# guy3540/Acoustic_Locating_VQ-VAE

Hardware: AMD Instinct MI355X
Metric: spectrograms/sec (train step), speech VQ-VAE default config (higher is better)
Workload: dtype x3mx_hb

## Files before the change

acoustic_locating_vq-vae_amd/csrc/pack_weights.hip:

```cpp
#include "alvq_common.h"
#include "bf16_common.h"
#include "f16mx_common.h"
#include "nlc_host.h"

namespace alvq {

constexpr int PB_MAX = 32;
struct PackDesc {
  const float* w;
  u16* wp;
  int M, C, KW, layout, Mp, Cp, blk0, ctiles;
};
struct PackBatch {
  PackDesc d[PB_MAX];
  int n;
  long plane[PB_MAX];
};

template <int PLANES>
__device__ __forceinline__ void pack_store8(u16* wp, long plane, long row_off, int c, const float (&v)[8]) {
  const long o = row_off + c;
  if (PLANES == 3) {
    unsigned h[4], qh[2], ql[2];
    fx_split<8>(v, fx_pow2(FX_E_W), fx_pow2(FX_E_W - FX_LO_SHIFT), h, qh, ql);
    *(u32x4*)(wp + o) = u32x4{h[0], h[1], h[2], h[3]};
    unsigned char* q = (unsigned char*)(wp + plane) + row_off * 2 + fx_q_off(c);
    *(u32x2*)q = u32x2{qh[0], qh[1]};
    *(u32x2*)(q + 32) = u32x2{ql[0], ql[1]};
    return;
  }
  u32x4 hi;
#pragma unroll
  for (int e = 0; e < 4; ++e) hi[e] = f2bf_pk(v[2 * e], v[2 * e + 1]);
  *(u32x4*)(wp + o) = hi;
  if (PLANES == 2) {
    u32x4 lo;
#pragma unroll
    for (int e = 0; e < 4; ++e) {
      const float h0 = __uint_as_float(hi[e] << 16), h1 = __uint_as_float(hi[e] & 0xffff0000u);
      lo[e] = f2bf_pk(v[2 * e] - h0, v[2 * e + 1] - h1);
    }
    *(u32x4*)(wp + plane + o) = lo;
  }
}

template <int PLANES>
__global__ __launch_bounds__(256) void pack_weights_batch_kernel(PackBatch b) {
  __shared__ float tile[3][32][65];
  if (PLANES == 3) fx_saturating_conversions();
  int di = 0;
  for (int i = 1; i < b.n; ++i)
    if ((int)blockIdx.x >= b.d[i].blk0) di = i;
  const PackDesc& d = b.d[di];
  const int lb = blockIdx.x - d.blk0;
  const int m0 = (lb / d.ctiles) * 32, c0 = (lb % d.ctiles) * 64;
  const int KW = d.KW, tid = threadIdx.x;
  if (d.layout == ALVQ_W_OIK) {
    const int run = 64 * KW;
#pragma unroll 4
    for (int e = tid; e < 32 * run; e += 256) {
      const int mr = e / run, j = e - mr * run, c = j / KW, t = j - c * KW;
      const int m = m0 + mr;
      tile[t][mr][c] = (m < d.M && c0 + c < d.C) ? d.w[((long)m * d.C + c0) * KW + j] : 0.f;
    }
  } else {
    const int run = 32 * KW;
#pragma unroll 4
    for (int e = tid; e < 64 * run; e += 256) {
      const int cc = e / run, j = e - cc * run, mr = j / KW, k = j - mr * KW;
      const int c = c0 + cc;
      tile[KW - 1 - k][mr][cc] = (c < d.C && m0 + mr < d.M) ? d.w[((long)c * d.M + m0) * KW + j] : 0.f;
    }
  }
  __syncthreads();
  const int mr = tid >> 3, cg = (tid & 7) * 8;
  for (int t = 0; t < KW; ++t) {
    float v[8];
#pragma unroll
    for (int e = 0; e < 8; ++e) v[e] = tile[t][mr][cg + e];
    pack_store8<PLANES>(d.wp, b.plane[di], ((long)t * d.Mp + m0 + mr) * d.Cp, c0 + cg, v);
  }
}

constexpr int AP_MAX = 24;
struct AdamPackDesc {
  float* w; const float* g; float* m; float* v;
  u16* oik; u16* iok;
  int dim0, dim1, KW, blk0, tiles1;
  int oik_Mp, oik_Cp, iok_Mp, iok_Cp;
};
struct AdamPackBatch {
  AdamPackDesc d[AP_MAX];
  int n;
  const float* sc;
  const float* skip;
  float beta1, beta2, eps;
};

template <int PLANES>
__global__ __launch_bounds__(256) void adam_pack_batch_kernel(AdamPackBatch b) {
  __shared__ float tile[3][32][65];
  if (b.skip && *b.skip != 0.f) return;
  if (PLANES == 3) fx_saturating_conversions();
  int di = 0;
  for (int i = 1; i < b.n; ++i)
    if ((int)blockIdx.x >= b.d[i].blk0) di = i;
  const AdamPackDesc& d = b.d[di];
  const int lb = blockIdx.x - d.blk0;
  const int r0 = (lb / d.tiles1) * 32, q0 = (lb % d.tiles1) * 64;
  const int KW = d.KW, tid = threadIdx.x;
  const float lr_bc1 = b.sc[0], bc2_sqrt = b.sc[1], gscale = b.sc[2];
  const float beta1 = b.beta1, beta2 = b.beta2, eps = b.eps;
  const int run = 64 * KW;
  if (q0 + 64 <= d.dim1 && ((d.dim1 * KW) & 3) == 0) {
#pragma unroll 2
    for (int e4 = tid; e4 < 8 * run; e4 += 256) {
      const int e = 4 * e4, rr = e / run, j = e - rr * run;
      f32x4 wn = {0.f, 0.f, 0.f, 0.f};
      if (r0 + rr < d.dim0) {
        const long i = ((long)(r0 + rr) * d.dim1 + q0) * KW + j;
        const f32x4 g4 = *(const f32x4*)(d.g + i), m4 = *(const f32x4*)(d.m + i), v4 = *(const f32x4*)(d.v + i), w4 = *(const f32x4*)(d.w + i);
        f32x4 mo, vo;
#pragma unroll
        for (int q = 0; q < 4; ++q) {
          const float gr = g4[q] * gscale;
          const float mm = m4[q] + (gr - m4[q]) * (1.f - beta1);
          const float vv = v4[q] * beta2 + (1.f - beta2) * gr * gr;
          const float denom = sqrtf(vv) / bc2_sqrt + eps;
          mo[q] = mm;
          vo[q] = vv;
          wn[q] = w4[q] - lr_bc1 * (mm / denom);
        }
        *(f32x4*)(d.m + i) = mo;
        *(f32x4*)(d.v + i) = vo;
        *(f32x4*)(d.w + i) = wn;
      }
#pragma unroll
      for (int q = 0; q < 4; ++q) {
        const int jj = j + q, qq = jj / KW, t = jj - qq * KW;
        tile[t][rr][qq] = wn[q];
      }
    }
  } else {
#pragma unroll 2
    for (int e = tid; e < 32 * run; e += 256) {
      const int rr = e / run, j = e - rr * run, qq = j / KW, t = j - qq * KW;
      float wn = 0.f;
      if (r0 + rr < d.dim0 && q0 + qq < d.dim1) {
        const long i = ((long)(r0 + rr) * d.dim1 + q0) * KW + j;
        const float gr = d.g[i] * gscale;
        const float m0 = d.m[i], v0 = d.v[i];
        const float mm = m0 + (gr - m0) * (1.f - beta1);
        const float vv = v0 * beta2 + (1.f - beta2) * gr * gr;
        const float denom = sqrtf(vv) / bc2_sqrt + eps;
        d.m[i] = mm;
        d.v[i] = vv;
        wn = d.w[i] - lr_bc1 * (mm / denom);
        d.w[i] = wn;
      }
      tile[t][rr][qq] = wn;
    }
  }
  __syncthreads();
  if (d.oik) {
    const int mr = tid >> 3, cg = (tid & 7) * 8;
    const long plane = (long)KW * d.oik_Mp * d.oik_Cp;
    for (int t = 0; t < KW; ++t) {
      float v[8];
#pragma unroll
      for (int e = 0; e < 8; ++e) v[e] = tile[t][mr][cg + e];
      pack_store8<PLANES>(d.oik, plane, ((long)t * d.oik_Mp + r0 + mr) * d.oik_Cp, q0 + cg, v);
    }
  }
  if (d.iok) {
    const int mr = tid >> 2, cg = (tid & 3) * 8;
    const long plane = (long)KW * d.iok_Mp * d.iok_Cp;
    for (int t = 0; t < KW; ++t) {
      float v[8];
#pragma unroll
      for (int e = 0; e < 8; ++e) v[e] = tile[KW - 1 - t][cg + e][mr];
      pack_store8<PLANES>(d.iok, plane, ((long)t * d.iok_Mp + q0 + mr) * d.iok_Cp, r0 + cg, v);
    }
  }
}

constexpr int AS_MAX = 48;
struct AdamSegs {
  long lo[AS_MAX], hi[AS_MAX];
  int blk0[AS_MAX];
  int n;
};
__global__ __launch_bounds__(256) void adam_segments_kernel(float* p, const float* g, float* m, float* v, AdamSegs s, const float* sc,
                                                            float beta1, float beta2, float eps, const float* skip) {
  if (skip && *skip != 0.f) return;
  int si = 0;
  for (int i = 1; i < s.n; ++i)
    if ((int)blockIdx.x >= s.blk0[i]) si = i;
  const float lr_bc1 = sc[0], bc2_sqrt = sc[1], gscale = sc[2];
  const long base = s.lo[si] + (long)(blockIdx.x - s.blk0[si]) * 1024;
#pragma unroll
  for (int k = 0; k < 4; ++k) {
    const long e = base + k * 256 + threadIdx.x;
    if (e >= s.hi[si]) return;
    const float gr = g[e] * gscale;
    const float mm = m[e] + (gr - m[e]) * (1.f - beta1);
    const float vv = v[e] * beta2 + (1.f - beta2) * gr * gr;
    const float denom = sqrtf(vv) / bc2_sqrt + eps;
    m[e] = mm;
    v[e] = vv;
    p[e] = p[e] - lr_bc1 * (mm / denom);
  }
}

}

using namespace alvq;

extern "C" int alvq_pack_weights_bf16_batch(const alvq_pack_desc* descs, int n, int planes, void* stream) {
  ALVQ_REQUIRE(descs && n > 0, ALVQ_EINVAL, "alvq_pack_weights_bf16_batch: no descriptors");
  ALVQ_REQUIRE(planes >= 1 && planes <= 3, ALVQ_EINVAL, "alvq_pack_weights_bf16_batch: planes=%d (1, 2 or 3)", planes);
  for (int i = 0; i < n; ++i) {
    const alvq_pack_desc& s = descs[i];
    ALVQ_REQUIRE(s.w && s.wp, ALVQ_EINVAL, "alvq_pack_weights_bf16_batch: null pointer in descriptor %d", i);
    ALVQ_REQUIRE(s.M > 0 && s.C > 0 && (s.KW == 1 || s.KW == 3), ALVQ_EINVAL, "alvq_pack_weights_bf16_batch: bad dims in descriptor %d", i);
    ALVQ_REQUIRE(s.w_layout == ALVQ_W_OIK || s.w_layout == ALVQ_W_IOK, ALVQ_EINVAL, "alvq_pack_weights_bf16_batch: w_layout in descriptor %d", i);
  }
  for (int i0 = 0; i0 < n; i0 += PB_MAX) {
    PackBatch b{};
    b.n = n - i0 < PB_MAX ? n - i0 : PB_MAX;
    int blocks = 0;
    for (int i = 0; i < b.n; ++i) {
      const alvq_pack_desc& s = descs[i0 + i];
      PackDesc& d = b.d[i];
      d.w = s.w; d.wp = (u16*)s.wp; d.M = s.M; d.C = s.C; d.KW = s.KW; d.layout = s.w_layout;
      d.Mp = pad_to(s.M, WP_ROWS); d.Cp = pad_to(s.C, TB_K);
      d.blk0 = blocks; d.ctiles = d.Cp / 64;
      b.plane[i] = (long)s.KW * d.Mp * d.Cp;
      blocks += (d.Mp / 32) * d.ctiles;
    }
    if (planes == 1) hipLaunchKernelGGL(pack_weights_batch_kernel<1>, dim3(blocks), dim3(256), 0, (hipStream_t)stream, b);
    else if (planes == 2) hipLaunchKernelGGL(pack_weights_batch_kernel<2>, dim3(blocks), dim3(256), 0, (hipStream_t)stream, b);
    else hipLaunchKernelGGL(pack_weights_batch_kernel<3>, dim3(blocks), dim3(256), 0, (hipStream_t)stream, b);
    int rc = check_launch("alvq_pack_weights_bf16_batch");
    if (rc) return rc;
  }
  return ALVQ_OK;
}

extern "C" int alvq_adam_pack_batch(const alvq_adam_pack_desc* descs, int n, int planes, const float* scalars, float beta1,
                                    float beta2, float eps, const float* skip, void* stream) {
  ALVQ_REQUIRE(descs && n > 0 && scalars, ALVQ_EINVAL, "alvq_adam_pack_batch: no descriptors / scalars");
  ALVQ_REQUIRE(planes >= 1 && planes <= 3, ALVQ_EINVAL, "alvq_adam_pack_batch: planes=%d (1, 2 or 3)", planes);
  for (int i = 0; i < n; ++i) {
    const alvq_adam_pack_desc& s = descs[i];
    ALVQ_REQUIRE(s.w && s.g && s.m && s.v, ALVQ_EINVAL, "alvq_adam_pack_batch: null pointer in descriptor %d", i);
    ALVQ_REQUIRE(s.dim0 > 0 && s.dim1 > 0 && (s.KW == 1 || s.KW == 3), ALVQ_EINVAL, "alvq_adam_pack_batch: bad dims in descriptor %d", i);
  }
  for (int i0 = 0; i0 < n; i0 += AP_MAX) {
    AdamPackBatch b{};
    b.n = n - i0 < AP_MAX ? n - i0 : AP_MAX;
    b.sc = scalars; b.skip = skip; b.beta1 = beta1; b.beta2 = beta2; b.eps = eps;
    int blocks = 0;
    for (int i = 0; i < b.n; ++i) {
      const alvq_adam_pack_desc& s = descs[i0 + i];
      AdamPackDesc& d = b.d[i];
      d.w = s.w; d.g = s.g; d.m = s.m; d.v = s.v; d.oik = (u16*)s.wp_oik; d.iok = (u16*)s.wp_iok;
      d.dim0 = s.dim0; d.dim1 = s.dim1; d.KW = s.KW;
      d.oik_Mp = pad_to(s.dim0, WP_ROWS); d.oik_Cp = pad_to(s.dim1, TB_K);
      d.iok_Mp = pad_to(s.dim1, WP_ROWS); d.iok_Cp = pad_to(s.dim0, TB_K);
      d.blk0 = blocks; d.tiles1 = (s.dim1 + 63) / 64;
      blocks += ((s.dim0 + 31) / 32) * d.tiles1;
    }
    if (planes == 1) hipLaunchKernelGGL(adam_pack_batch_kernel<1>, dim3(blocks), dim3(256), 0, (hipStream_t)stream, b);
    else if (planes == 2) hipLaunchKernelGGL(adam_pack_batch_kernel<2>, dim3(blocks), dim3(256), 0, (hipStream_t)stream, b);
    else hipLaunchKernelGGL(adam_pack_batch_kernel<3>, dim3(blocks), dim3(256), 0, (hipStream_t)stream, b);
    int rc = check_launch("alvq_adam_pack_batch");
    if (rc) return rc;
  }
  return ALVQ_OK;
}

extern "C" int alvq_adam_segments_f32(float* param, const float* grad, float* exp_avg, float* exp_avg_sq, const int64_t* lo,
                                      const int64_t* hi, int nseg, const float* scalars, float beta1, float beta2, float eps,
                                      const float* skip, void* stream) {
  ALVQ_REQUIRE(param && grad && exp_avg && exp_avg_sq && scalars && lo && hi, ALVQ_EINVAL, "alvq_adam_segments_f32: null pointer");
  ALVQ_REQUIRE(nseg > 0, ALVQ_EINVAL, "alvq_adam_segments_f32: no segments");
  for (int i0 = 0; i0 < nseg; i0 += AS_MAX) {
    AdamSegs s{};
    s.n = nseg - i0 < AS_MAX ? nseg - i0 : AS_MAX;
    int blocks = 0;
    for (int i = 0; i < s.n; ++i) {
      ALVQ_REQUIRE(lo[i0 + i] >= 0 && hi[i0 + i] > lo[i0 + i], ALVQ_EINVAL, "alvq_adam_segments_f32: bad segment %d", i0 + i);
      s.lo[i] = lo[i0 + i]; s.hi[i] = hi[i0 + i];
      s.blk0[i] = blocks;
      blocks += (int)((hi[i0 + i] - lo[i0 + i] + 1023) / 1024);
    }
    hipLaunchKernelGGL(adam_segments_kernel, dim3(blocks), dim3(256), 0, (hipStream_t)stream, param, grad, exp_avg, exp_avg_sq, s, scalars,
                       beta1, beta2, eps, skip);
    int rc = check_launch("alvq_adam_segments_f32");
    if (rc) return rc;
  }
  return ALVQ_OK;
}
```

acoustic_locating_vq-vae_amd/csrc/wgrad_reduce_batch.hip:

```cpp
#include "alvq_common.h"
#include "wgrad_reduce.h"

namespace alvq {

constexpr int RB_MAX = 40;
struct ReduceBatch {
  alvq_reduce_desc d[RB_MAX];
  int blk0[RB_MAX];
  int nblk[RB_MAX];
  int n;
};

__global__ __launch_bounds__(256) void wgrad_reduce_batch_kernel(ReduceBatch b) {
  __shared__ float tile[3][16][65];
  int di = 0;
  for (int i = 1; i < b.n; ++i)
    if ((int)blockIdx.x >= b.blk0[i]) di = i;
  const alvq_reduce_desc& d = b.d[di];
  const int lb = blockIdx.x - b.blk0[di];
  const int acc = d.accumulate;
  if (d.w_layout == ALVQ_W_IOK && d.stride == (int64_t)d.KW * d.M * d.C)
    wgrad_reduce_iok_body<16>(tile, d.partial, d.dst, d.splits, d.KW, d.M, d.C, acc, d.scale, lb);
  else
    wgrad_reduce_body(d.partial, d.dst, d.splits, d.KW, d.M, d.C, d.w_layout, acc, d.scale, (long)d.stride, lb, b.nblk[di]);
}

}

using namespace alvq;

extern "C" int alvq_wgrad_reduce_batch(const alvq_reduce_desc* descs, int n, void* stream) {
  ALVQ_REQUIRE(descs && n > 0, ALVQ_EINVAL, "alvq_wgrad_reduce_batch: no descriptors");
  for (int i = 0; i < n; ++i) {
    const alvq_reduce_desc& s = descs[i];
    ALVQ_REQUIRE(s.partial && s.dst, ALVQ_EINVAL, "alvq_wgrad_reduce_batch: null pointer in descriptor %d", i);
    ALVQ_REQUIRE(s.splits >= 1 && s.splits <= 64 && s.M > 0 && s.C > 0 && (s.KW == 1 || s.KW == 3), ALVQ_EINVAL,
                 "alvq_wgrad_reduce_batch: bad dims in descriptor %d", i);
    ALVQ_REQUIRE(s.w_layout == ALVQ_W_OIK || s.w_layout == ALVQ_W_IOK, ALVQ_EINVAL, "alvq_wgrad_reduce_batch: w_layout in descriptor %d", i);
    ALVQ_REQUIRE(s.stride >= (int64_t)s.KW * s.M * s.C, ALVQ_EINVAL, "alvq_wgrad_reduce_batch: stride in descriptor %d", i);
  }
  for (int i0 = 0; i0 < n; i0 += RB_MAX) {
    ReduceBatch b{};
    b.n = n - i0 < RB_MAX ? n - i0 : RB_MAX;
    int blocks = 0;
    for (int i = 0; i < b.n; ++i) {
      const alvq_reduce_desc& s = descs[i0 + i];
      b.d[i] = s;
      const long total = (long)s.KW * s.M * s.C;
      int nb;
      if (s.w_layout == ALVQ_W_IOK && s.stride == total) nb = ((s.M + 15) / 16) * ((s.C + 63) / 64);
      else {
        nb = (int)((total + 255) / 256);
        if (nb > 2048) nb = 2048;
      }
      b.blk0[i] = blocks;
      b.nblk[i] = nb;
      blocks += nb;
    }
    hipLaunchKernelGGL(wgrad_reduce_batch_kernel, dim3(blocks), dim3(256), 0, (hipStream_t)stream, b);
    int rc = check_launch("alvq_wgrad_reduce_batch");
    if (rc) return rc;
  }
  return ALVQ_OK;
}
```

Measured before the change: 7677.

## Vectorize wgrad split reduction and batch Adam loads with nontemporal streaming

The batched weight-gradient reduction gains float4-vectorized bodies for OIK (flat) and IOK (tiled) layouts. Each thread sums several splits with batched loads. Descriptors are sorted by estimated per-block work so heavy blocks launch first, and block lookup uses binary search. The fused Adam+pack kernel is specialized on kernel width, batches several float4 loads before computing, and uses nontemporal loads and stores for gradient and moment buffers, aiming to raise memory-level parallelism and cut cache pollution. The cost is more code paths and higher register use.

```diff
diff --git a/acoustic_locating_vq-vae_amd/csrc/pack_weights.hip b/acoustic_locating_vq-vae_amd/csrc/pack_weights.hip
--- a/acoustic_locating_vq-vae_amd/csrc/pack_weights.hip
+++ b/acoustic_locating_vq-vae_amd/csrc/pack_weights.hip
@@ -83,11 +83,13 @@
 }
 
 constexpr int AP_MAX = 24;
+constexpr int AP_ROWS = 32;
 struct AdamPackDesc {
   float* w; const float* g; float* m; float* v;
   u16* oik; u16* iok;
   int dim0, dim1, KW, blk0, tiles1;
   int oik_Mp, oik_Cp, iok_Mp, iok_Cp;
+  int vec;
 };
 struct AdamPackBatch {
   AdamPackDesc d[AP_MAX];
@@ -97,53 +99,64 @@
   float beta1, beta2, eps;
 };
 
-template <int PLANES>
-__global__ __launch_bounds__(256) void adam_pack_batch_kernel(AdamPackBatch b) {
-  __shared__ float tile[3][32][65];
-  if (b.skip && *b.skip != 0.f) return;
-  if (PLANES == 3) fx_saturating_conversions();
-  int di = 0;
-  for (int i = 1; i < b.n; ++i)
-    if ((int)blockIdx.x >= b.d[i].blk0) di = i;
-  const AdamPackDesc& d = b.d[di];
-  const int lb = blockIdx.x - d.blk0;
-  const int r0 = (lb / d.tiles1) * 32, q0 = (lb % d.tiles1) * 64;
-  const int KW = d.KW, tid = threadIdx.x;
+__device__ __forceinline__ f32x4 ap_load_stream(const float* p) { return __builtin_nontemporal_load((const f32x4*)p); }
+__device__ __forceinline__ void ap_store_stream(float* p, f32x4 v) { __builtin_nontemporal_store(v, (f32x4*)p); }
+
+template <int KW>
+__device__ __forceinline__ void adam_tile(const AdamPackBatch& b, const AdamPackDesc& d, float (&tile)[3][AP_ROWS][65], int r0, int q0) {
+  const int tid = threadIdx.x;
   const float lr_bc1 = b.sc[0], bc2_sqrt = b.sc[1], gscale = b.sc[2];
   const float beta1 = b.beta1, beta2 = b.beta2, eps = b.eps;
-  const int run = 64 * KW;
-  if (q0 + 64 <= d.dim1 && ((d.dim1 * KW) & 3) == 0) {
-#pragma unroll 2
-    for (int e4 = tid; e4 < 8 * run; e4 += 256) {
-      const int e = 4 * e4, rr = e / run, j = e - rr * run;
-      f32x4 wn = {0.f, 0.f, 0.f, 0.f};
-      if (r0 + rr < d.dim0) {
-        const long i = ((long)(r0 + rr) * d.dim1 + q0) * KW + j;
-        const f32x4 g4 = *(const f32x4*)(d.g + i), m4 = *(const f32x4*)(d.m + i), v4 = *(const f32x4*)(d.v + i), w4 = *(const f32x4*)(d.w + i);
-        f32x4 mo, vo;
+  constexpr int run = 64 * KW;
+  if (d.vec && q0 + 64 <= d.dim1) {
+    constexpr int NV = AP_ROWS * run / 4 / 256, BATCH = KW == 3 ? 3 : (NV < 4 ? NV : 4);
+    static_assert(NV % BATCH == 0, "tile / batch");
+    for (int it0 = 0; it0 < NV; it0 += BATCH) {
+      f32x4 g4[BATCH], m4[BATCH], v4[BATCH], w4[BATCH];
+      long idx[BATCH];
+      int rrs[BATCH], js[BATCH];
+#pragma unroll
+      for (int u = 0; u < BATCH; ++u) {
+        const int e = 4 * (tid + 256 * (it0 + u));
+        rrs[u] = e / run;
+        js[u] = e - rrs[u] * run;
+        idx[u] = ((long)(r0 + rrs[u]) * d.dim1 + q0) * KW + js[u];
+        if (r0 + rrs[u] < d.dim0) {
+          g4[u] = ap_load_stream(d.g + idx[u]);
+          m4[u] = ap_load_stream(d.m + idx[u]);
+          v4[u] = ap_load_stream(d.v + idx[u]);
+          w4[u] = *(const f32x4*)(d.w + idx[u]);
+        }
+      }
+#pragma unroll
+      for (int u = 0; u < BATCH; ++u) {
+        f32x4 wn = {0.f, 0.f, 0.f, 0.f};
+        if (r0 + rrs[u] < d.dim0) {
+          f32x4 mo, vo;
+#pragma unroll
+          for (int q = 0; q < 4; ++q) {
+            const float gr = g4[u][q] * gscale;
+            const float mm = m4[u][q] + (gr - m4[u][q]) * (1.f - beta1);
+            const float vv = v4[u][q] * beta2 + (1.f - beta2) * gr * gr;
+            const float denom = sqrtf(vv) / bc2_sqrt + eps;
+            mo[q] = mm;
+            vo[q] = vv;
+            wn[q] = w4[u][q] - lr_bc1 * (mm / denom);
+          }
+          ap_store_stream(d.m + idx[u], mo);
+          ap_store_stream(d.v + idx[u], vo);
+          *(f32x4*)(d.w + idx[u]) = wn;
+        }
 #pragma unroll
         for (int q = 0; q < 4; ++q) {
-          const float gr = g4[q] * gscale;
-          const float mm = m4[q] + (gr - m4[q]) * (1.f - beta1);
-          const float vv = v4[q] * beta2 + (1.f - beta2) * gr * gr;
-          const float denom = sqrtf(vv) / bc2_sqrt + eps;
-          mo[q] = mm;
-          vo[q] = vv;
-          wn[q] = w4[q] - lr_bc1 * (mm / denom);
+          const int jj = js[u] + q, qq = jj / KW, t = jj - qq * KW;
+          tile[t][rrs[u]][qq] = wn[q];
         }
-        *(f32x4*)(d.m + i) = mo;
-        *(f32x4*)(d.v + i) = vo;
-        *(f32x4*)(d.w + i) = wn;
-      }
-#pragma unroll
-      for (int q = 0; q < 4; ++q) {
-        const int jj = j + q, qq = jj / KW, t = jj - qq * KW;
-        tile[t][rr][qq] = wn[q];
       }
     }
   } else {
 #pragma unroll 2
-    for (int e = tid; e < 32 * run; e += 256) {
+    for (int e = tid; e < AP_ROWS * run; e += 256) {
       const int rr = e / run, j = e - rr * run, qq = j / KW, t = j - qq * KW;
       float wn = 0.f;
       if (r0 + rr < d.dim0 && q0 + qq < d.dim1) {
@@ -161,25 +174,46 @@
       tile[t][rr][qq] = wn;
     }
   }
+}
+
+template <int PLANES>
+__global__ __launch_bounds__(256) void adam_pack_batch_kernel(AdamPackBatch b) {
+  __shared__ float tile[3][AP_ROWS][65];
+  if (b.skip && *b.skip != 0.f) return;
+  if (PLANES == 3) fx_saturating_conversions();
+  int di = 0;
+  for (int i = 1; i < b.n; ++i)
+    if ((int)blockIdx.x >= b.d[i].blk0) di = i;
+  const AdamPackDesc& d = b.d[di];
+  const int lb = blockIdx.x - d.blk0;
+  const int r0 = (lb / d.tiles1) * AP_ROWS, q0 = (lb % d.tiles1) * 64;
+  const int KW = d.KW, tid = threadIdx.x;
+  if (KW == 3) adam_tile<3>(b, d, tile, r0, q0);
+  else adam_tile<1>(b, d, tile, r0, q0);
   __syncthreads();
   if (d.oik) {
-    const int mr = tid >> 3, cg = (tid & 7) * 8;
     const long plane = (long)KW * d.oik_Mp * d.oik_Cp;
-    for (int t = 0; t < KW; ++t) {
-      float v[8];
-#pragma unroll
-      for (int e = 0; e < 8; ++e) v[e] = tile[t][mr][cg + e];
-      pack_store8<PLANES>(d.oik, plane, ((long)t * d.oik_Mp + r0 + mr) * d.oik_Cp, q0 + cg, v);
+    for (int u = tid; u < AP_ROWS * 8; u += 256) {
+      const int mr = u >> 3, cg = (u & 7) * 8;
+      for (int t = 0; t < KW; ++t) {
+        float v[8];
+#pragma unroll
+        for (int e = 0; e < 8; ++e) v[e] = tile[t][mr][cg + e];
+        pack_store8<PLANES>(d.oik, plane, ((long)t * d.oik_Mp + r0 + mr) * d.oik_Cp, q0 + cg, v);
+      }
     }
   }
   if (d.iok) {
-    const int mr = tid >> 2, cg = (tid & 3) * 8;
+    constexpr int CG = AP_ROWS / 8;
     const long plane = (long)KW * d.iok_Mp * d.iok_Cp;
-    for (int t = 0; t < KW; ++t) {
-      float v[8];
-#pragma unroll
-      for (int e = 0; e < 8; ++e) v[e] = tile[KW - 1 - t][cg + e][mr];
-      pack_store8<PLANES>(d.iok, plane, ((long)t * d.iok_Mp + q0 + mr) * d.iok_Cp, r0 + cg, v);
+    for (int u = tid; u < 64 * CG; u += 256) {
+      const int mr = u / CG, cg = (u % CG) * 8;
+      for (int t = 0; t < KW; ++t) {
+        float v[8];
+#pragma unroll
+        for (int e = 0; e < 8; ++e) v[e] = tile[KW - 1 - t][cg + e][mr];
+        pack_store8<PLANES>(d.iok, plane, ((long)t * d.iok_Mp + q0 + mr) * d.iok_Cp, r0 + cg, v);
+      }
     }
   }
 }
@@ -268,8 +302,9 @@
       d.dim0 = s.dim0; d.dim1 = s.dim1; d.KW = s.KW;
       d.oik_Mp = pad_to(s.dim0, WP_ROWS); d.oik_Cp = pad_to(s.dim1, TB_K);
       d.iok_Mp = pad_to(s.dim1, WP_ROWS); d.iok_Cp = pad_to(s.dim0, TB_K);
+      d.vec = ((((uintptr_t)s.w | (uintptr_t)s.g | (uintptr_t)s.m | (uintptr_t)s.v) & 15) == 0 && ((long)s.dim1 * s.KW) % 4 == 0) ? 1 : 0;
       d.blk0 = blocks; d.tiles1 = (s.dim1 + 63) / 64;
-      blocks += ((s.dim0 + 31) / 32) * d.tiles1;
+      blocks += ((s.dim0 + AP_ROWS - 1) / AP_ROWS) * d.tiles1;
     }
     if (planes == 1) hipLaunchKernelGGL(adam_pack_batch_kernel<1>, dim3(blocks), dim3(256), 0, (hipStream_t)stream, b);
     else if (planes == 2) hipLaunchKernelGGL(adam_pack_batch_kernel<2>, dim3(blocks), dim3(256), 0, (hipStream_t)stream, b);
diff --git a/acoustic_locating_vq-vae_amd/csrc/wgrad_reduce_batch.hip b/acoustic_locating_vq-vae_amd/csrc/wgrad_reduce_batch.hip
--- a/acoustic_locating_vq-vae_amd/csrc/wgrad_reduce_batch.hip
+++ b/acoustic_locating_vq-vae_amd/csrc/wgrad_reduce_batch.hip
@@ -1,28 +1,131 @@
+#include <algorithm>
+
 #include "alvq_common.h"
 #include "wgrad_reduce.h"
 
 namespace alvq {
 
 constexpr int RB_MAX = 40;
+enum ReduceBody : int { RB_SCALAR = 0, RB_IOK_TILE = 1, RB_FLAT4 = 2, RB_IOK_TILE4 = 3 };
 struct ReduceBatch {
   alvq_reduce_desc d[RB_MAX];
-  int blk0[RB_MAX];
-  int nblk[RB_MAX];
+  int blk0[RB_MAX + 1];
+  int body[RB_MAX];
   int n;
 };
 
+template <int KW, int N>
+static __device__ __forceinline__ void add_splits(f32x4 (&s)[KW], const float* p, int k, long stride, long plane) {
+  f32x4 v[N][KW];
+#pragma unroll
+  for (int u = 0; u < N; ++u)
+#pragma unroll
+    for (int t = 0; t < KW; ++t) v[u][t] = *(const f32x4*)(p + (long)(k + u) * stride + (long)t * plane);
+#pragma unroll
+  for (int u = 0; u < N; ++u)
+#pragma unroll
+    for (int t = 0; t < KW; ++t) s[t] += v[u][t];
+}
+template <int KW>
+static __device__ __forceinline__ void sum_splits(f32x4 (&s)[KW], const float* p, int splits, long stride, long plane) {
+  constexpr int U = KW == 3 ? 4 : 8;
+#pragma unroll
+  for (int t = 0; t < KW; ++t) s[t] = f32x4{0.f, 0.f, 0.f, 0.f};
+  int k = 0;
+  for (; k + U <= splits; k += U) add_splits<KW, U>(s, p, k, stride, plane);
+  if (U == 8 && k + 4 <= splits) { add_splits<KW, 4>(s, p, k, stride, plane); k += 4; }
+  if (k + 2 <= splits) { add_splits<KW, 2>(s, p, k, stride, plane); k += 2; }
+  if (k < splits) add_splits<KW, 1>(s, p, k, stride, plane);
+}
+
+template <int KW>
+static __device__ __forceinline__ void reduce_flat4_body(const float* partial, float* dw, int splits, long pairs, long stride,
+                                                         int accumulate, const float* scale, int bid) {
+  const long q4 = bid * 256L + threadIdx.x;
+  if (q4 >= (pairs >> 2)) return;
+  f32x4* o = (f32x4*)(dw + 4 * KW * q4);
+  f32x4 old[KW];
+  if (accumulate) {
+#pragma unroll
+    for (int j = 0; j < KW; ++j) old[j] = o[j];
+  }
+  f32x4 s[KW];
+  sum_splits<KW>(s, partial + 4 * q4, splits, stride, pairs);
+  float r[4 * KW];
+#pragma unroll
+  for (int i = 0; i < 4; ++i)
+#pragma unroll
+    for (int t = 0; t < KW; ++t) r[i * KW + t] = s[t][i];
+  if (scale) {
+    const float sc = *scale;
+#pragma unroll
+    for (int j = 0; j < 4 * KW; ++j) r[j] *= sc;
+  }
+#pragma unroll
+  for (int j = 0; j < KW; ++j) {
+    f32x4 v = {r[4 * j], r[4 * j + 1], r[4 * j + 2], r[4 * j + 3]};
+    if (accumulate) v += old[j];
+    o[j] = v;
+  }
+}
+
+template <int KW>
+static __device__ __forceinline__ void reduce_iok4_body(float (&tile)[3][16][65], const float* partial, float* dw, int splits, int M,
+                                                        int C, long stride, int accumulate, const float* scale, int bid) {
+  const int ctiles = (C + 63) / 64;
+  const int m0 = (bid / ctiles) * 16, c0 = (bid % ctiles) * 64;
+  const int tx = threadIdx.x & 15, ty = threadIdx.x >> 4;
+  const int m = m0 + ty, c = c0 + 4 * tx;
+  f32x4 s[KW];
+  if (m < M && c < C) sum_splits<KW>(s, partial + (long)m * C + c, splits, stride, (long)M * C);
+  else {
+#pragma unroll
+    for (int t = 0; t < KW; ++t) s[t] = f32x4{0.f, 0.f, 0.f, 0.f};
+  }
+#pragma unroll
+  for (int t = 0; t < KW; ++t)
+#pragma unroll
+    for (int i = 0; i < 4; ++i) tile[t][ty][4 * tx + i] = s[t][i];
+  __syncthreads();
+  constexpr int run = 16 * KW;
+  for (int e = threadIdx.x; e < 64 * run; e += 256) {
+    const int cc = e / run, j = e - cc * run, mr = j / KW, tt = j - mr * KW;
+    if (c0 + cc >= C || m0 + mr >= M) continue;
+    const long o = ((long)(c0 + cc) * M + m0) * KW + j;
+    float v = tile[KW - 1 - tt][mr][cc];
+    if (scale) v *= *scale;
+    dw[o] = accumulate ? dw[o] + v : v;
+  }
+}
+
 __global__ __launch_bounds__(256) void wgrad_reduce_batch_kernel(ReduceBatch b) {
   __shared__ float tile[3][16][65];
-  int di = 0;
-  for (int i = 1; i < b.n; ++i)
-    if ((int)blockIdx.x >= b.blk0[i]) di = i;
+  int di = 0, hi = b.n;
+  while (hi - di > 1) {
+    const int mid = (di + hi) >> 1;
+    if ((int)blockIdx.x >= b.blk0[mid]) di = mid;
+    else hi = mid;
+  }
   const alvq_reduce_desc& d = b.d[di];
   const int lb = blockIdx.x - b.blk0[di];
   const int acc = d.accumulate;
-  if (d.w_layout == ALVQ_W_IOK && d.stride == (int64_t)d.KW * d.M * d.C)
-    wgrad_reduce_iok_body<16>(tile, d.partial, d.dst, d.splits, d.KW, d.M, d.C, acc, d.scale, lb);
-  else
-    wgrad_reduce_body(d.partial, d.dst, d.splits, d.KW, d.M, d.C, d.w_layout, acc, d.scale, (long)d.stride, lb, b.nblk[di]);
+  const long pairs = (long)d.M * d.C;
+  switch (b.body[di]) {
+    case RB_FLAT4:
+      if (d.KW == 3) reduce_flat4_body<3>(d.partial, d.dst, d.splits, pairs, (long)d.stride, acc, d.scale, lb);
+      else reduce_flat4_body<1>(d.partial, d.dst, d.splits, pairs, (long)d.stride, acc, d.scale, lb);
+      break;
+    case RB_IOK_TILE4:
+      if (d.KW == 3) reduce_iok4_body<3>(tile, d.partial, d.dst, d.splits, d.M, d.C, (long)d.stride, acc, d.scale, lb);
+      else reduce_iok4_body<1>(tile, d.partial, d.dst, d.splits, d.M, d.C, (long)d.stride, acc, d.scale, lb);
+      break;
+    case RB_IOK_TILE:
+      wgrad_reduce_iok_body<16>(tile, d.partial, d.dst, d.splits, d.KW, d.M, d.C, acc, d.scale, lb);
+      break;
+    default:
+      wgrad_reduce_body(d.partial, d.dst, d.splits, d.KW, d.M, d.C, d.w_layout, acc, d.scale, (long)d.stride, lb,
+                        b.blk0[di + 1] - b.blk0[di]);
+  }
 }
 
 }
@@ -40,23 +143,46 @@
     ALVQ_REQUIRE(s.stride >= (int64_t)s.KW * s.M * s.C, ALVQ_EINVAL, "alvq_wgrad_reduce_batch: stride in descriptor %d", i);
   }
   for (int i0 = 0; i0 < n; i0 += RB_MAX) {
+    const int cnt = n - i0 < RB_MAX ? n - i0 : RB_MAX;
+    int body[RB_MAX], nblk[RB_MAX], order[RB_MAX];
+    long work[RB_MAX];
+    for (int i = 0; i < cnt; ++i) {
+      const alvq_reduce_desc& s = descs[i0 + i];
+      const long pairs = (long)s.M * s.C, total = s.KW * pairs;
+      const bool al16 = (((uintptr_t)s.partial | (uintptr_t)s.dst) & 15) == 0 && (s.stride & 3) == 0;
+      const int tiles = ((s.M + 15) / 16) * ((s.C + 63) / 64);
+      if (s.w_layout == ALVQ_W_OIK && al16 && (pairs & 3) == 0) {
+        body[i] = RB_FLAT4;
+        nblk[i] = (int)((pairs / 4 + 255) / 256);
+        work[i] = 4096L * s.KW * s.splits;
+      } else if (s.w_layout == ALVQ_W_IOK && al16 && (s.C & 3) == 0) {
+        body[i] = RB_IOK_TILE4;
+        nblk[i] = tiles;
+        work[i] = 4096L * s.KW * s.splits;
+      } else if (s.w_layout == ALVQ_W_IOK && s.stride == total) {
+        body[i] = RB_IOK_TILE;
+        nblk[i] = tiles;
+        work[i] = 4096L * s.KW * s.splits;
+      } else {
+        body[i] = RB_SCALAR;
+        nblk[i] = (int)((total + 255) / 256);
+        if (nblk[i] > 2048) nblk[i] = 2048;
+        work[i] = total * 4 * s.splits / nblk[i];
+      }
+      order[i] = i;
+    }
+    std::stable_sort(order, order + cnt, [&](int a, int c) { return work[a] > work[c]; });
     ReduceBatch b{};
-    b.n = n - i0 < RB_MAX ? n - i0 : RB_MAX;
+    b.n = cnt;
     int blocks = 0;
-    for (int i = 0; i < b.n; ++i) {
-      const alvq_reduce_desc& s = descs[i0 + i];
-      b.d[i] = s;
-      const long total = (long)s.KW * s.M * s.C;
-      int nb;
-      if (s.w_layout == ALVQ_W_IOK && s.stride == total) nb = ((s.M + 15) / 16) * ((s.C + 63) / 64);
-      else {
-        nb = (int)((total + 255) / 256);
-        if (nb > 2048) nb = 2048;
-      }
-      b.blk0[i] = blocks;
-      b.nblk[i] = nb;
-      blocks += nb;
+    for (int j = 0; j < cnt; ++j) {
+      const int i = order[j];
+      b.d[j] = descs[i0 + i];
+      b.body[j] = body[i];
+      b.blk0[j] = blocks;
+      blocks += nblk[i];
     }
+    b.blk0[cnt] = blocks;
     hipLaunchKernelGGL(wgrad_reduce_batch_kernel, dim3(blocks), dim3(256), 0, (hipStream_t)stream, b);
     int rc = check_launch("alvq_wgrad_reduce_batch");
     if (rc) return rc;
```

After: 7692, median of 6. No clear change (+0.2%).
